# drscotthawley/flocoder

Hardware: NVIDIA B200
Metric: samples/sec, 50-step RK4 latent sampling (higher is better)
Workload: dtype bf16

## Files before the change

### flocoder_b200/csrc/api.cu

```cuda
#include <cuda_fp16.h>
#include <math.h>
#include <stdarg.h>
#include <stdio.h>
#include <stdlib.h>
#include <string.h>

#include <algorithm>
#include <chrono>
#include <float.h>
#include <map>
#include <memory>
#include <string>
#include <vector>

#include "flo_internal.h"

namespace flo {

int conv_umma_smem_bytes(const ConvUmmaParams& p);

static thread_local std::string g_last_error;
void set_error(const char* fmt, ...) {
    char buf[1024];
    va_list ap;
// ... 1535 lines not shown
        } else {
            snprintf(line, sizeof(line), "%3zu %-7s %-28s in=%s out_m=%s out_o=%s\n", i, kinds[op.kind], op.name.c_str(), bn(op.gn_in),
                     bn(op.out_m), bn(op.out_o));
            t += line;
        }
    }
    for (size_t i = 0; i < h.bufs.size(); ++i) {
        const Buf& bf = h.bufs[i];
        snprintf(line, sizeof(line), "buf %3zu %-34s C=%d %dx%d %s bytes_ps=%zu live=[%d,%d] off_ps=%zu\n", i, bf.name.c_str(), bf.C, bf.H,
                 bf.W, bf.bf16 ? "bf16" : "f32 ", bf.bytes_ps, bf.def, bf.last, bf.off_ps);
        t += line;
    }
    if (h.spec.fused) {
        FusedBuilder fb(h, h.ftensors, h.fstages, 4);
        rc = fb.build();
        if (rc) return rc;
        snprintf(line, sizeof(line), "fused: %d stages, %d boundary tensors, %zu bytes/sample\n", (int)h.fstages.size(),
                 (int)h.ftensors.size(), h.farena_ps);
        t += line;
        for (size_t i = 0; i < h.fstages.size(); ++i) {
            const FStage& st = h.fstages[i];
            if (st.kind == 0) {
                const ChainParams& c = st.cp;
                snprintf(line, sizeof(line), "stage %2zu chain %-12s %dx%d nb=%d mt=%d strips=%d steps=%d loads=%d smem=%d (slots %d, ring %dx%d) tmem=%d nsplit=%d ctas=%d\n",
                         i, st.name.c_str(), c.H, c.W, c.nb, c.n_mtiles, c.strips, c.n_steps, c.n_loads, c.smem_bytes, c.ring_off,
                         c.n_ring, c.ring_slot_bytes, c.tmem_cols, c.nsplit, c.nsplit * ((B + c.nb - 1) / c.nb));
                t += line;
                for (int k = 0; k < c.n_steps; ++k) {
                    const ChainStep& cs = c.st[k];
                    snprintf(line, sizeof(line), "      step %d: conv=%d k=%d cin=%d+%d n=%d chunks=%dx%d res=%d(%dx%d) epi=%d C=%d G=%d film=%d resmode=%d out_slot=%d out_g=%d un=%d up=%d pn=%d final=%d a0=%d a1=%d\n",
                             k, cs.has_conv, cs.ksize, cs.a0_ncb * 8, cs.a1_ncb * 8, cs.n, cs.slices, cs.slices_per_chunk, cs.has_res,
                             cs.res_slices, cs.res_slices_per_chunk, cs.epi, cs.C, cs.groups, cs.film_off, cs.res_mode, cs.out_slot_off,
                             cs.out_g, cs.out_un_g, cs.out_up_g, cs.pn_g, cs.final, cs.a0_off, cs.a1_off);
                    t += line;
                }
            } else {
                const AttnFusedParams& a = st.ap;
                snprintf(line, sizeof(line), "stage %2zu attn  %-12s %dx%d C=%d nb=%d n=%d n_pad=%d mt=%d full=%d smem=%d plane=%d tmem=%d cols(k=%d v=%d ctx=%d q=%d out=%d proj=%d) ctas=%d\n",
                         i, st.name.c_str(), a.H, a.W, a.C, a.nb, a.n, a.n_pad, a.n_mtiles, a.full, a.smem_bytes, a.plane_bytes, a.tmem_cols,
                         a.col_k, a.col_v, a.col_ctx, a.col_q, a.col_out, a.col_proj, (B + a.nb - 1) / a.nb);
                t += line;
            }
        }
        for (size_t i = 0; i < h.ftensors.size(); ++i) {
            snprintf(line, sizeof(line), "ftensor %2zu %-24s C=%d %dx%d off_ps=%zu\n", i, h.ftensors[i].name.c_str(), h.ftensors[i].C,
                     h.ftensors[i].H, h.ftensors[i].W, h.ftensors[i].off_ps);
            t += line;
        }
    }
    if (out && cap > 0) snprintf(out, cap, "%s", t.c_str());
    return (int)t.size();
}

static void op_cost(const Handle& h, const Op& op, double& fl, double& by) {
    const Spec& s = h.spec;
// ... 212 lines not shown
```

### flocoder_b200/csrc/flo_internal.h

```cpp
#pragma once
#include <cuda_runtime.h>
#include <cuda_bf16.h>
#include <cuda.h>
#include <stdint.h>
#include <string>
#include <vector>

#include "../../include/flocoder_b200.h"

namespace flo {

enum StageKind : int {
    ST_PLAIN = 0,
    ST_RK1 = 1,
    ST_RK2 = 2,
    ST_RK3 = 3,
    ST_RK4 = 4,
    ST_EULER = 5,
    ST_CFG_COND = 6,
    ST_STORE = 7
};
enum StageFlags : int {
    SF_CFG_COMBINE = 1,
    SF_CFG_2B = 2
// ... 169 lines not shown
size_t pack_umma_weights(const float* w_oihw, int cout, int cin, int ksize, const int* perm, int n_tile, bool f16,
                         std::vector<__nv_bfloat16>& out);

typedef CUresult (*EncodeTiledFn)(CUtensorMap*, CUtensorMapDataType, cuuint32_t, void*, const cuuint64_t*,
                                  const cuuint64_t*, const cuuint32_t*, const cuuint32_t*, CUtensorMapInterleave,
                                  CUtensorMapSwizzle, CUtensorMapL2promotion, CUtensorMapFloatOOBfill);
EncodeTiledFn get_encode_tiled();

void set_error(const char* fmt, ...);

constexpr int MAX_WSTAGES = 8;
constexpr int CH_MAX_STEPS = 8;
constexpr int CH_MAX_LOADS = 4;
constexpr int CH_MAX_GT = 10;
enum ChainEpi : int { CE_GN = 1, CE_BIAS = 2, CE_INIT = 3 };

struct ChainStep {
    int has_conv;
    int a0_off, a0_ncb, a1_off, a1_ncb;
    int ksize, n;
    int acc_col;
    unsigned w_off; int slices, slices_per_chunk;
    int has_res, res_col; unsigned wres_off; int res_slices, res_slices_per_chunk;
    int tab_idx, res_tab_idx;
    int chunk0, res_chunk0;
    int epi;
    int C, groups, silu, film_off;
    int bias_off, gamma_off, beta_off;
    int res_mode;
    int res_slot_off, res_bias_off;
    int out_slot_off;
    int out_g, out_un_g, out_up_g;
    int pn_g, pn_gamma_off, pn_beta_off;
    int final;
};

struct ChainParams {
    int n_steps;
    ChainStep st[CH_MAX_STEPS];
    int B, H, W, nb, n_mtiles, strips, plane_px;
    int n_loads, load_off[CH_MAX_LOADS], load_ncb[CH_MAX_LOADS];
    int zero_off, zero_bytes;
    int ones_off;
    int fast;
    int max_c;
    int g_max, coef_n, cpar_n;
    int wide;
    int ring_off, ring_slot_bytes, n_ring, n_ring_deep;
    int stats_off, bar_off, smem_bytes, tmem_cols;
    int tab_off, tab_n;
    int wtab_off, n_chunks;
    int tabs_off;
    int nsplit;
    int xpart_off;
    int fmt;
    int film_dim;
    int cin0, dim, channels;
    int init_w_off, init_b_off, final_w_off, final_b_off;
    const uint16_t* wblob;
    const float* fblob;
    void* gt[CH_MAX_GT];
    Ctrl* ctrl;
    long long* dbg;
};

struct AttnFusedParams {
    int epi_warps;
    int B, H, W, C, nb, n, n_pad, n_mtiles;
    int full;
    int ktrans;
    int small;
    int fmt;
    unsigned wq_off, wk_off, wv_off, wo_off;
    int qkv_chunks, qkv_S, o_chunks, o_S;
    int bo_off, gamma_off, beta_off;
    int xh_off, p_off, v_off, ct_off, kmax_off, stats_off;
    int plane_bytes;
// ... 54 lines not shown
```

### flocoder_b200/csrc/fused.cu

```cuda
#include <cuda_fp16.h>

#include <cstring>
#include <type_traits>
#include "flo_internal.h"
#include "umma_common.cuh"
#include "fused_common.cuh"

namespace flo {

struct Geo {
    int W, H, Wp, PP, nb, B, strips, sbo_px, tx_n;
};
__device__ __forceinline__ Geo make_geo(const ChainParams& p) {
    Geo g;
    g.W = p.W; g.H = p.H; g.Wp = p.W + 2; g.PP = g.Wp * (p.H + 2); g.nb = p.nb; g.B = p.B;
    g.strips = p.strips; g.sbo_px = p.strips ? g.Wp : 8; g.tx_n = p.W >> 3;
    return g;
}
__device__ __forceinline__ int tile_row0(const Geo& g, int t) {
    if (g.strips) return ((t / g.tx_n) * 16 + 1) * g.Wp + 1 + 8 * (t % g.tx_n);
    return g.Wp + 1 + t * 128;
}
struct RowInfo {
    int pp;
    int s, px;
    bool valid;
};
__device__ __forceinline__ RowInfo make_row(const Geo& g, int t, int r, int b0) {
    RowInfo ri;
    ri.pp = tile_row0(g, t) + (r >> 3) * g.sbo_px + (r & 7);
    ri.s = ri.pp / g.PP;
    const int rem = ri.pp - ri.s * g.PP;
    const int hh = rem / g.Wp, ww = rem - hh * g.Wp;
    ri.px = (hh - 1) * g.W + (ww - 1);
    ri.valid = (ri.s < g.nb) && (b0 + ri.s < g.B) && hh >= 1 && hh <= g.H && ww >= 1 && ww <= g.W;
    return ri;
}

struct RingPos {
    int slot; uint32_t phase;
    __device__ __forceinline__ void next(int n_ring) { if (++slot == n_ring) { slot = 0; phase ^= 1u; } }
};
struct ConvIssue {
    const int32_t* tab;
    int n, col, slices, S;
};
template <int MT>
struct IssueCtx {
    uint32_t tmem_base, bar_full, bar_empty, ring_lo, ring_slot16, ones_lo;
    uint32_t plane16;
    uint32_t desc_hi_a, desc_hi_ones;
    int n_ring;
    uint32_t row0[MT];
    int cc;
    RingPos rp;
    long long* dbg;
};
__device__ __forceinline__ uint64_t desc64(uint32_t lo, uint32_t hi) {
    uint64_t d;
    asm("mov.b64 %0, {%1, %2};" : "=l"(d) : "r"(lo), "r"(hi));
    return d;
}
template <int MT, int FMT>
__device__ __forceinline__ void issue_conv(IssueCtx<MT>& x, const ConvIssue& c) {
    const uint32_t idesc = make_idesc16(128, c.n, FMT, 0, 0);
    const uint32_t b_hi = (128u >> 4) | (1u << 14);
    const uint32_t b_lbo = ((uint32_t)c.n & 0x3FFFu) << 16;
    const uint32_t a_lbo = (x.plane16 & 0x3FFFu) << 16;
    const uint32_t slice16 = (uint32_t)c.n * 2u;
    const int conv_slices = c.slices - 1;
    for (int ks0 = 0; ks0 < c.slices; ks0 += c.S) {
        const int cnt = min(c.S, c.slices - ks0);
        const int slot = x.rp.slot;
        mbar_wait(x.bar_full + 8 * slot, x.rp.phase);
        tc_fence_after();
        if (x.dbg && x.cc >= 8 && x.cc < 16 && (threadIdx.x & 31) == 0) x.dbg[104 + (x.cc - 8) * 3 + 2] = clock64();
        if (elect_one()) {
            uint32_t b_lo = (x.ring_lo + (uint32_t)slot * x.ring_slot16) | b_lbo;
            const int32_t* tp = c.tab + ks0;
            const int n_conv = min(cnt, conv_slices - ks0);
            uint32_t acc = ks0 > 0 ? 1u : 0u;
            auto mma_slice = [&](int32_t e) {
                const uint64_t bdesc = desc64(b_lo, b_hi);
                const uint32_t a_base = (uint32_t)e | a_lbo;
#pragma unroll
                for (int t = 0; t < MT; ++t)
                    umma_bf16(x.tmem_base + (uint32_t)(c.col + t * c.n), desc64(a_base + x.row0[t], x.desc_hi_a), bdesc, idesc, acc);
                acc = 1u;
                b_lo += slice16;
            };
            int s = 0;
            if constexpr (MT == 1) {
                int32_t e[4], f[4];
#pragma unroll
                for (int k = 0; k < 4; ++k) e[k] = (n_conv >= 4) ? tp[k] : 0;
                for (; s + 4 <= n_conv; s += 4) {
#pragma unroll
                    for (int k = 0; k < 4; ++k) f[k] = (s + 8 <= n_conv) ? tp[s + 4 + k] : 0;
#pragma unroll
                    for (int k = 0; k < 4; ++k) mma_slice(e[k]);
#pragma unroll
                    for (int k = 0; k < 4; ++k) e[k] = f[k];
                }
            } else {
                int32_t cur = n_conv > 0 ? tp[0] : 0;
                for (; s < n_conv; ++s) {
                    const int32_t nxt = tp[s + 1];
                    mma_slice(cur);
                    cur = nxt;
                }
            }
            for (; s < n_conv; ++s) mma_slice(tp[s]);
            if (ks0 + cnt == c.slices) {
                const uint64_t bdesc = desc64(b_lo, b_hi);
                const uint64_t adesc = desc64(x.ones_lo | (8u << 16), x.desc_hi_ones);
#pragma unroll
                for (int t = 0; t < MT; ++t) umma_bf16(x.tmem_base + (uint32_t)(c.col + t * c.n), adesc, bdesc, idesc, 1u);
            }
            umma_commit(x.bar_empty + 8 * slot);
        }
        __syncwarp();
        ++x.cc;
        x.rp.next(x.n_ring);
    }
}

template <int N> struct IntTag { static constexpr int value = N; };

struct XChg {
    int nsplit; uint32_t rank, smem_base, bar_x; int xpart_off; uint32_t* phase; uint8_t* smem;
};
__device__ __forceinline__ void stats_to_coef(const Geo& g, int R, const float2* rowstat, float2* coef, const float2* gpar, int G, int pm,
                                              int C, int HW, bool has_film, int et, const XChg* xc = nullptr) {
    const int lgG = 31 - __clz(G), combos = g.nb * G, cpg = C >> lgG, GS = G * pm;
    const int cpw = (combos + EPI_WARPS - 1) / EPI_WARPS;
    int seg = 32;
// ... 57 lines not shown
        }
    }
    epi_sync();
}

template <int NV>
__device__ __forceinline__ int warp_sum_scatter(float (&p)[NV], int lane) {
    int idx = 0, o = 16;
#pragma unroll
    for (int h = NV / 2; h >= 1; h >>= 1, o >>= 1) {
        const bool upper = (lane & o) != 0;
#pragma unroll
        for (int j = 0; j < h; ++j) {
            const float send = upper ? p[j] : p[j + h];
            const float keep = upper ? p[j + h] : p[j];
            p[j] = keep + __shfl_xor_sync(0xffffffffu, send, o);
        }
        idx += upper ? h : 0;
    }
    for (; o >= 1; o >>= 1) p[0] += __shfl_xor_sync(0xffffffffu, p[0], o);
    return idx;
}

#ifndef FLO_CHAIN_MINB
#define FLO_CHAIN_MINB 2
#endif
constexpr int FINAL_MAX_CH = 4;
template <int MT, bool SPLIT, int FMT, bool FAST, bool WIDE = false, int ENDS = 3>
__global__ void __launch_bounds__(FUSED_THREADS, (MT <= 2 && !SPLIT && !WIDE) ? FLO_CHAIN_MINB : 1) k_chain(const __grid_constant__ CUtensorMap tm0,
                                                         const __grid_constant__ CUtensorMap tm1,
                                                         const __grid_constant__ CUtensorMap tm2,
                                                         const __grid_constant__ CUtensorMap tm3,
                                                         const __grid_constant__ ChainParams p) {
    extern __shared__ __align__(128) uint8_t smem[];
    const int warp = threadIdx.x >> 5, lane = threadIdx.x & 31, tid = threadIdx.x;
    constexpr int W_PROD = EPI_WARPS, W_MMA = EPI_WARPS + 1;
    const uint32_t smem_base = smem_u32(smem);
    const int bar_off = p.bar_off;
    const uint32_t bar_full = smem_base + bar_off;
    const uint32_t bar_empty = bar_full + 8 * MAX_WSTAGES;
    const uint32_t bar_load = bar_empty + 8 * MAX_WSTAGES;
    const uint32_t bar_mma = bar_load + 8;
    const uint32_t bar_epi = bar_mma + 8;
    const uint32_t tmem_slot = bar_epi + 8;
    const uint32_t bar_x = tmem_slot + 8;
    const uint32_t bar_epi2 = bar_x + 8;
    volatile uint32_t* tmem_slot_ptr = reinterpret_cast<volatile uint32_t*>(smem + bar_off + 16 * MAX_WSTAGES + 24);
    const Geo geo = make_geo(p);
    const int Q = SPLIT ? p.nsplit : 1;
    const uint32_t qrank = SPLIT ? cluster_ctarank() : 0u;
    const int lgQ = SPLIT ? 31 - __clz(Q) : 0;
    const int b0 = ((int)blockIdx.x >> lgQ) * geo.nb;
    const uint32_t plane_bytes = (uint32_t)p.plane_px * 16u;
    const int n_steps = p.n_steps, n_ring = p.n_ring, n_loads = p.n_loads, tmem_cols = p.tmem_cols;
    const int ones_off = p.ones_off;
    long long* dbg = (blockIdx.x == 0) ? p.dbg : nullptr;
    if (p.dbg && tid == 0 && blockIdx.x == 0) p.dbg[100] = global_ns();

    if (warp == W_PROD && lane == 0) {
        for (int i = 0; i < n_ring; ++i) { mbar_init(bar_full + 8 * i, 1); mbar_init(bar_empty + 8 * i, 1); }
        mbar_init(bar_load, 1);
        mbar_init(bar_mma, 1);
        mbar_init(bar_epi, SPLIT ? 1 : EPI_THREADS);
        mbar_init(bar_epi2, 1);
        mbar_init(bar_x, SPLIT ? 1 : EPI_THREADS);
        asm volatile("fence.mbarrier_init.release.cluster;" ::: "memory");
    }
    if (warp == W_MMA) tmem_alloc(tmem_slot, (uint32_t)tmem_cols);
    {
        const int zoff = p.zero_off, zbytes = p.zero_bytes;
        for (int i = tid * 16; i < zbytes; i += FUSED_THREADS * 16) *reinterpret_cast<uint4*>(smem + zoff + i) = make_uint4(0, 0, 0, 0);
        const uint32_t ones2 = pack2t<FMT>(1.0f, 1.0f);
        for (int i = tid; i < 256; i += FUSED_THREADS)
            *reinterpret_cast<uint4*>(smem + ones_off + i * 16) = make_uint4(i < 128 ? ones2 : 0u, 0, 0, 0);
    }
    int32_t* atab = reinterpret_cast<int32_t*>(smem + p.tab_off);
    {
        const int32_t* gtab = reinterpret_cast<const int32_t*>(p.fblob + p.tabs_off);
        const int base16 = (int)((smem_base >> 4) & 0x3FFFu);
        const int tab_n = p.tab_n, n_chunks = p.n_chunks;
        for (int i = tid; i < tab_n; i += FUSED_THREADS) atab[i] = gtab[i] + base16;
        const uint2* gw = reinterpret_cast<const uint2*>(gtab + tab_n) + (size_t)qrank * n_chunks;
        uint2* wtab_w = reinterpret_cast<uint2*>(smem + p.wtab_off);
        for (int i = tid; i < n_chunks; i += FUSED_THREADS) wtab_w[i] = gw[i];
    }
    fence_proxy_async();
    tc_fence_before();
    if (Q > 1) cluster_sync_all();
    else __syncthreads();
    tc_fence_after();
    const uint32_t tmem_base = *tmem_slot_ptr;
    if (dbg && tid == 0) dbg[CH_MAX_STEPS * 8] = clock64();
    if (dbg && tid == 0) dbg[101] = global_ns();

    if (warp == W_PROD) {
        if (dbg && lane == 8) {
            for (int cc = 0; cc < 16 && cc < p.n_chunks; ++cc) {
                mbar_wait(bar_full + 8 * (cc % n_ring), (uint32_t)(cc / n_ring) & 1u);
                if (cc >= 8) dbg[104 + (cc - 8) * 3] = clock64();
            }
        }
        constexpr int NL = 2;
        if (lane < NL) {
            const uint32_t ring_base = smem_base + p.ring_off, ring_slot_bytes = p.ring_slot_bytes;
            const uint2* wtab = reinterpret_cast<const uint2*>(smem + p.wtab_off);
// ... 29 lines not shown
        x.plane16 = plane_bytes >> 4;
        x.desc_hi_a = (((uint32_t)geo.sbo_px * 16u) >> 4) | (1u << 14);
        x.desc_hi_ones = (128u >> 4) | (1u << 14);
        x.n_ring = n_ring; x.cc = 0; x.rp.slot = 0; x.rp.phase = 0; x.dbg = dbg;
#pragma unroll
        for (int t = 0; t < MT; ++t) x.row0[t] = (uint32_t)(tile_row0(geo, t) - (geo.Wp + 1));
        if (n_loads > 0) mbar_wait(bar_load, 0);
        for (int i = 0; i < n_steps; ++i) {
            if (i > 0) {
                if (SPLIT) {
                    const int live = min(geo.nb, geo.B - b0) * geo.H * geo.W;
                    const uint32_t bar = ((i - 1) & 1) ? bar_epi2 : bar_epi;
                    if (elect_one()) mbar_expect_tx(bar, (uint32_t)(live * (p.st[i - 1].C >> 3) * 16));
                    __syncwarp();
                    mbar_wait_cluster(bar, ((i - 1) >> 1) & 1);
                    fence_proxy_async_all();
                } else {
                    named_bar_sync(2, EPI_THREADS + 32);
                }
            }
            tc_fence_after();
            if (dbg && lane == 0) dbg[i * 8 + 0] = clock64();
            if (p.st[i].has_conv) {
                ConvIssue c;
                c.tab = atab + p.st[i].tab_idx;
                c.n = p.st[i].n; c.col = p.st[i].acc_col; c.slices = p.st[i].slices;
                c.S = p.st[i].slices_per_chunk;
                issue_conv<MT, FMT>(x, c);
                if (p.st[i].has_res) {
                    c.tab = atab + p.st[i].res_tab_idx;
                    c.col = p.st[i].res_col; c.slices = p.st[i].res_slices; c.S = p.st[i].res_slices_per_chunk;
                    issue_conv<MT, FMT>(x, c);
                }
                if (dbg && lane == 0) dbg[i * 8 + 1] = clock64();
                if (elect_one()) umma_commit(bar_mma);
            } else {
                if (elect_one()) mbar_arrive(bar_mma);
            }
            __syncwarp();
        }
    } else {
        const int wg = warp >> 2, quad = warp & 3;
        const int r = quad * 32 + lane;
        const int et = tid;
        const uint32_t tlane = tmem_base + ((uint32_t)(quad * 32) << 16);
        float2* rowstat = reinterpret_cast<float2*>(smem + p.stats_off);
        float2* coef = rowstat + MT * 128 * p.g_max;
        float* cpar = reinterpret_cast<float*>(coef + p.coef_n);
        const int cpar_n = p.cpar_n;
        float2* gpar = reinterpret_cast<float2*>(cpar + cpar_n);
        float* const fastbuf = reinterpret_cast<float*>(gpar + p.max_c);
        Ctrl* ctrl = p.ctrl;
        const float* fblob = p.fblob;
        const int HW = geo.H * geo.W;
// ... 9 lines not shown
            const int t = (MT == 1) ? 0 : wg + 2 * k;
            if (t < MT) ri[k] = make_row(geo, t, r, b0);
            else { ri[k].pp = 0; ri[k].s = 0; ri[k].px = 0; ri[k].valid = false; }
        }
        if (n_loads > 0) mbar_wait(bar_load, 0);
        uint32_t xphase = 0;
        XChg xc;
        xc.nsplit = Q; xc.rank = qrank; xc.smem_base = smem_base; xc.bar_x = bar_x; xc.xpart_off = p.xpart_off; xc.phase = &xphase;
        xc.smem = smem;

        for (int i = 0; i < n_steps; ++i) {
            const int epi = p.st[i].epi, Ctot = p.st[i].C, acc_col = p.st[i].acc_col, res_col = p.st[i].res_col;
            const int C = Ctot >> lgQ, c0 = (int)qrank * C;
            const int res_mode = p.st[i].res_mode, res_slot_off = p.st[i].res_slot_off;
            const int is_final = (ENDS & 2) ? p.st[i].final : 0, pn_g = p.st[i].pn_g;
            const int out_slot_off = p.st[i].out_slot_off;
            uint4* const og = p.st[i].out_g >= 0 ? reinterpret_cast<uint4*>(p.gt[p.st[i].out_g]) : nullptr;
            int cbeg = 0, cend = C;
            if (MT == 1) {
                if (is_final) { cend = wg == 0 ? C : 0; }
                else { cbeg = wg * (C >> 1); cend = cbeg + (C >> 1); }
            }
            const bool cw8 = (cend - cbeg) == 8;
            auto write8 = [&](const RowInfo& R, int cb, const float* v8) -> uint4 {
                const uint4 u = pack8t<FMT>(v8);
                if (out_slot_off >= 0) {
                    const uint32_t soff = (uint32_t)out_slot_off + (uint32_t)cb * plane_bytes + (uint32_t)R.pp * 16u;
                    if (!SPLIT) *reinterpret_cast<uint4*>(smem + soff) = u;
                    else if (i + 1 < n_steps) {
                        const uint32_t bar = (i & 1) ? bar_epi2 : bar_epi;
                        for (int q = 0; q < Q; ++q) st_async_v4(mapa_shared(smem_base + soff, (uint32_t)q), u, mapa_shared(bar, (uint32_t)q));
                    } else {
                        *reinterpret_cast<uint4*>(smem + soff) = u;
                    }
                }
                if (og) og[(size_t)(cb * geo.B + b0 + R.s) * HW + R.px] = u;
                return u;
            };
            auto for_chunks = [&](auto&& fn) {
                if (cw8) {
                    fn(0, cbeg, IntTag<8>());
                } else {
#pragma unroll
                    for (int k = 0; k < TW; ++k) {
                        if (MT > 1 && wg + 2 * k >= MT) continue;
                        for (int c = cbeg; c < cend; c += 16) fn(k, c, IntTag<16>());
// ... 184 lines not shown
                    const int b = b0 + ri[k].s;
                    float xin[16];
#pragma unroll
                    for (int ci = 0; ci < 16; ++ci) xin[ci] = ci < cin0 ? xs[((size_t)b * cin0 + ci) * HW + ri[k].px] : 0.f;
                    for (int c8 = cbeg; c8 < cend; c8 += 8) {
                        float v[8];
#pragma unroll
                        for (int j = 0; j < 8; ++j) {
                            float a = cpar[C * cin0 + c8 + j];
                            if (cin0 == 4) {
                                const float4 w4 = *reinterpret_cast<const float4*>(cpar + (c8 + j) * 4);
                                a = fmaf(xin[0], w4.x, a); a = fmaf(xin[1], w4.y, a); a = fmaf(xin[2], w4.z, a); a = fmaf(xin[3], w4.w, a);
                            } else {
#pragma unroll
                                for (int ci = 0; ci < 16; ++ci)
                                    if (ci < cin0) a = fmaf(xin[ci], cpar[(c8 + j) * cin0 + ci], a);
                            }
                            v[j] = a;
                        }
                        write8(ri[k], (c0 + c8) >> 3, v);
                    }
                }
            } else if (epi == CE_BIAS) {
                for_chunks([&](int k, int c, auto tag) {
                    constexpr int CW = decltype(tag)::value;
                    uint32_t u[CW];
                    const uint32_t ta = tlane + (uint32_t)(acc_col + tile_of(k) * C + c);
                    if constexpr (CW == 16) tmem_ld16_issue(ta, u); else tmem_ld8_issue(ta, u);
                    tmem_ld_wait();
                    if (!ri[k].valid) return;
                    float v[CW];
#pragma unroll
                    for (int j = 0; j < CW; ++j) v[j] = __uint_as_float(u[j]);
#pragma unroll
                    for (int hb = 0; hb < CW / 8; ++hb) write8(ri[k], ((c0 + c) >> 3) + hb, v + hb * 8);
                });
            } else {
                const int G = p.st[i].groups >> lgQ, lg_cpg = 31 - __clz(C) - (31 - __clz(G)), cpg = 1 << lg_cpg;
                float kacc[TW][FINAL_MAX_CH];
                float psx[TW], psq[TW];
#pragma unroll
                for (int k = 0; k < TW; ++k) {
                    psx[k] = 0.f; psq[k] = 0.f;
#pragma unroll
                    for (int j = 0; j < FINAL_MAX_CH; ++j) kacc[k][j] = 0.f;
                }
                if constexpr (fast_gn_k) {
// ... 140 lines not shown
                                unpack8t<FMT>(pk[hb], xv);
                                const float4* pp4 = reinterpret_cast<const float4*>(pnpar + cbeg + hb * 8);
#pragma unroll
                                for (int j = 0; j < 8; j += 2) {
                                    const float4 gb = pp4[j >> 1];
                                    const float a0 = rstd * gb.x, a1 = rstd * gb.z;
                                    xv[j] = fmaf(xv[j], a0, gb.y - mean * a0); xv[j + 1] = fmaf(xv[j + 1], a1, gb.w - mean * a1);
                                }
                                dst[(size_t)(gcb * geo.B + b0) * HW + ri[0].px] = pack8t<FMT>(xv);
                            }
                        }
                    }
                } else {
                const int pm = (MT == 1 && G == 1 && !is_final) ? 2 : 1;
                const int GS = G * pm;
                bool fast2 = false;
                if constexpr (SPLIT && MT == 1)
                    fast2 = G == 1 && geo.PP == 16 && !is_final && (cend - cbeg == 8 || cend - cbeg == 16);
                bool fast3 = false;
                if constexpr (!SPLIT && MT == 1 && WIDE)
                    fast3 = geo.H == 4 && geo.W == 4 && geo.nb <= 3 && !is_final && (cpg == 8 || cpg == 16) && ((cend - cbeg) & 15) == 0 &&
                            cend > cbeg;
                if (fast2) {
                    if (dbg && et == 0) dbg[i * 8 + 3] = clock64();
                    auto body = [&](auto cw_tag) {
                        constexpr int CW = decltype(cw_tag)::value;
                        uint32_t av[CW];
                        const uint32_t ta = tlane + (uint32_t)(acc_col + cbeg);
                        if constexpr (CW == 16) tmem_ld16_issue(ta, av); else tmem_ld8_issue(ta, av);
                        tmem_ld_wait();
                        const bool valid = ri[0].valid;
                        float s0 = 0.f, q0 = 0.f, s1 = 0.f, q1 = 0.f;
#pragma unroll
                        for (int j = 0; j < CW; j += 2) {
                            const float xa = __uint_as_float(av[j]), xb = __uint_as_float(av[j + 1]);
                            s0 += xa; q0 = fmaf(xa, xa, q0); s1 += xb; q1 = fmaf(xb, xb, q1);
                        }
                        float sx = valid ? s0 + s1 : 0.f, sq = valid ? q0 + q1 : 0.f;
#pragma unroll
                        for (int o = 8; o > 0; o >>= 1) { sx += __shfl_xor_sync(0xffffffffu, sx, o); sq += __shfl_xor_sync(0xffffffffu, sq, o); }
                        float2* const part = reinterpret_cast<float2*>(fastbuf);
                        const int sl = r >> 4;
                        if ((lane & 15) == 0) part[wg * 8 + sl] = make_float2(sx, sq);
                        epi_sync();
                        if (dbg && et == 0) dbg[i * 8 + 4] = clock64();
                        uint32_t rv[CW];
                        if (res_mode == 1) {
                            const uint32_t tr = tlane + (uint32_t)(res_col + cbeg);
                            if constexpr (CW == 16) tmem_ld16_issue(tr, rv); else tmem_ld8_issue(tr, rv);
                            tmem_ld_wait();
                        }
                        if (!valid) return;
                        const float2 pa = part[sl], pb = part[8 + sl];
// ... 362 lines not shown
```

### flocoder_b200/csrc/fused_plan.inc

```

struct FusedBuilder {
    Handle& h;
    const Spec& s;
    std::vector<FTensor>& T;
    std::vector<FStage>& S;
    bool debug;
    int qcap;
    FusedBuilder(Handle& hh, std::vector<FTensor>& t, std::vector<FStage>& st, int qcap_)
        : h(hh), s(hh.spec), T(t), S(st), debug((hh.spec.flags & FLO_FLAG_NO_BUFFER_REUSE) != 0), qcap(qcap_) {}

    int tensor(const std::string& name, int C, int H, int W) {
        for (size_t i = 0; i < T.size(); ++i)
            if (T[i].name == name) return (int)i;
        FTensor t; t.name = name; t.C = C; t.H = H; t.W = W;
        t.bytes_ps = ((size_t)C * H * W * 2 + 255) & ~(size_t)255; t.off_ps = 0;
        T.push_back(t);
        return (int)T.size() - 1;
    }
    const Op& op(const std::string& name, int kind) {
        for (auto& o : h.ops)
            if (o.name == name && o.kind == kind) return o;
        set_error("internal: no op '%s'", name.c_str());
        throw 1;
    }
// ... 104 lines not shown
        }
        set_error("internal: global tensor table overflow in stage %s", cur.name.c_str());
        throw 1;
    }
    int load(int tensor_id) {
        const FTensor& t = T[tensor_id];
        const int off = slot(t.C);
        ChainParams& c = cur.cp;
        c.load_off[c.n_loads] = off; c.load_ncb[c.n_loads] = t.C / 8;
        cur.map_tensor[c.n_loads] = tensor_id;
        ++c.n_loads; cur.n_maps = c.n_loads;
        return off;
    }
    void mark_epi_slots() { if (first_epi_slot < 0) first_epi_slot = slot_top; }
    ChainStep& new_step() {
        ChainParams& c = cur.cp;
        if (c.n_steps >= CH_MAX_STEPS) { set_error("internal: too many steps in stage %s", cur.name.c_str()); throw 1; }
        ChainStep& st = c.st[c.n_steps++];
        memset(&st, 0, sizeof(st));
        st.film_off = -1; st.bias_off = -1; st.gamma_off = -1; st.beta_off = -1; st.res_slot_off = -1; st.res_bias_off = -1;
        st.out_slot_off = -1; st.out_g = -1; st.out_un_g = -1; st.out_up_g = -1; st.pn_g = -1;
        return st;
    }
    void set_conv(ChainStep& st, const Op& conv, int a0_off, int a0_C, int a1_off, int a1_C) {
        st.has_conv = 1;
        st.a0_off = a0_off; st.a0_ncb = a0_C / 8; st.a1_off = a1_off < 0 ? 0 : a1_off; st.a1_ncb = a1_off < 0 ? 0 : a1_C / 8;
        const int Q = cur.cp.nsplit, nq = conv.cout / Q;
        st.ksize = conv.ksize; st.n = nq; st.acc_col = 0;
        st.w_off = fused_stream(conv, Q);
        st.slices = conv.ksize * conv.ksize * (a0_C + (a1_off < 0 ? 0 : a1_C)) / 16 + 1;
        st.slices_per_chunk = chunk_slices(st.slices, nq);
        ring_slot = std::max(ring_slot, st.slices_per_chunk * nq * 32);
        max_n = std::max(max_n, nq);
        st.bias_off = -1;
        st.C = conv.cout;
    }
    int conv_bias(const std::string& opname, int a0_off, int a0_C, int C_out, int out_tensor = -1) {
        const Op& conv = op(opname, OP_CONV);
        mark_epi_slots();
        ChainStep& st = new_step();
        set_conv(st, conv, a0_off, a0_C, -1, 0);
        st.epi = CE_BIAS;
        st.out_slot_off = slot(C_out);
        st.out_g = gt(out_tensor);
        return st.out_slot_off;
    }
    int resblock(const std::string& p, int x0_off, int x0_C, int x1_off, int x1_C, int dout, int out_tensor, int pn_tensor,
                 bool is_final, int H, int W) {
        mark_epi_slots();
        const int cin = x0_C + (x1_off < 0 ? 0 : x1_C);
        const Op& c1 = op(p + ".block1.proj", OP_CONV);
        const Op& g1 = op(p + ".block1", OP_GN);
        if ((dout & (dout - 1)) || (g1.groups & (g1.groups - 1))) {
            set_error("fused path: channels (%d) and GroupNorm groups (%d) of '%s' must be powers of two", dout, g1.groups, p.c_str());
            throw 2;
        }
        const Op& c2 = op(p + ".block2.proj", OP_CONV);
        const Op& g2 = op(p, OP_GN);
        const bool has_res = cin != dout;
        const int hslot = slot(dout);
        {
            ChainStep& st = new_step();
            set_conv(st, c1, x0_off, x0_C, x1_off, x1_C);
            if (has_res) {
                const Op& rc = op(p + ".res_conv", OP_CONV);
                const int Q = cur.cp.nsplit;
                st.has_res = 1; st.wres_off = fused_stream(rc, Q);
                st.res_slices = cin / 16 + 1;
                st.res_slices_per_chunk = chunk_slices(st.res_slices, dout / Q);
                ring_slot = std::max(ring_slot, st.res_slices_per_chunk * (dout / Q) * 32);
            }
            st.epi = CE_GN; st.groups = g1.groups; st.silu = 1; st.film_off = g1.film_off;
            max_g = std::max(max_g, g1.groups); max_c = std::max(max_c, dout);
            st.gamma_off = (int)g1.gamma; st.beta_off = (int)g1.beta;
            st.out_slot_off = hslot;
            if (debug) st.out_g = gt(tensor(p + ".block1", dout, H, W));
        }
        int oslot = -1;
        {
            ChainStep& st = new_step();
            set_conv(st, c2, hslot, dout, -1, 0);
            st.epi = CE_GN; st.groups = g2.groups; st.silu = 1; st.film_off = -1;
            st.gamma_off = (int)g2.gamma; st.beta_off = (int)g2.beta;
            if (has_res) {
                st.res_mode = 1; st.res_bias_off = -1;
            } else {
                st.res_mode = 2; st.res_slot_off = x0_off;
            }
            if (is_final) {
                st.final = 1;
            } else {
                oslot = slot(dout);
                st.out_slot_off = oslot;
                st.out_g = gt(out_tensor);
                if (pn_tensor >= 0) {
                    const Op& pn = op(pn_name, OP_GN);
                    st.pn_g = gt(pn_tensor); st.pn_gamma_off = (int)pn.gamma; st.pn_beta_off = (int)pn.beta;
                }
            }
        }
        release(hslot, dout);
        return oslot;
    }
    std::string pn_name;
    int end_chain() {
        ChainParams& c = cur.cp;
        const int acc_cols = c.n_mtiles * max_n;
        bool any_res = false;
        for (int i = 0; i < c.n_steps; ++i) any_res |= c.st[i].has_res != 0;
        for (int i = 0; i < c.n_steps; ++i) {
            c.st[i].res_col = acc_cols;
            if (c.st[i].res_mode == 1) c.st[i].res_col = acc_cols;
        }
        int cols = 32;
        while (cols < acc_cols * (any_res ? 2 : 1)) cols <<= 1;
        if (cols > 512) { set_error("stage %s needs %d TMEM columns", cur.name.c_str(), cols); return FLO_ERR_UNSUPPORTED; }
        c.tmem_cols = cols;
        if (first_epi_slot < 0) first_epi_slot = slot_top;
        c.zero_off = first_epi_slot; c.zero_bytes = slot_top - first_epi_slot;
        const int Wp = c.W + 2;
        int off = (slot_top + (128 + Wp + 2) * 16 + 127) & ~127;
        c.ones_off = off; off += 4096;
        c.ring_slot_bytes = (ring_slot + 127) & ~127;
        c.g_max = std::max(max_g, 2); c.coef_n = c.nb * max_c;
        c.cpar_n = std::max(512, s.dim * (s.channels + 1));
        c.max_c = max_c;
        {
            bool fast = c.nb == 1 && c.n_mtiles <= 2 && c.nsplit == 1;
            for (int i = 0; i < c.n_steps && fast; ++i) {
                const int width = c.n_mtiles == 1 ? (c.st[i].final ? c.st[i].C : c.st[i].C / 2) : c.st[i].C;
                if (width > 16) fast = false;
            }
            c.fast = fast ? 1 : 0;
        }
        const int stats_bytes = (c.n_mtiles * 128 * c.g_max + c.coef_n) * 8 + c.cpar_n * 4 + max_c * 8 + 512 + 4 * max_c * 8;
        int tab_n = 0;
        for (int i = 0; i < c.n_steps; ++i) {
            if (!c.st[i].has_conv) continue;
            c.st[i].tab_idx = tab_n; tab_n += c.st[i].slices + 1;
            if (c.st[i].has_res) { c.st[i].res_tab_idx = tab_n; tab_n += c.st[i].res_slices + 1; }
        }
        c.tab_n = (tab_n + 3) & ~3;
        int n_chunks = 0;
        for (int i = 0; i < c.n_steps; ++i) {
            if (!c.st[i].has_conv) continue;
            c.st[i].chunk0 = n_chunks; n_chunks += (c.st[i].slices + c.st[i].slices_per_chunk - 1) / c.st[i].slices_per_chunk;
            if (c.st[i].has_res) {
                c.st[i].res_chunk0 = n_chunks;
                n_chunks += (c.st[i].res_slices + c.st[i].res_slices_per_chunk - 1) / c.st[i].res_slices_per_chunk;
            }
        }
        c.n_chunks = n_chunks;
        {
            std::vector<int32_t> tabs((size_t)c.tab_n + (size_t)c.nsplit * n_chunks * 2, 0);
            const int two_planes = (c.plane_px * 16 >> 4) * 2, Wp_ = c.W + 2;
            auto fill_a = [&](int idx, int conv_slices, int ksize, const ChainStep& st) {
                const int a0p = st.a0_ncb >> 1, pairs = a0p + (st.a1_ncb >> 1);
                for (int ks = 0; ks < conv_slices; ++ks) {
                    const int tap = ks / pairs, cp = ks - tap * pairs;
                    const int shift = (ksize == 3 ? ((tap / 3 - 1) * Wp_ + (tap % 3 - 1)) : 0) + Wp_ + 1;
                    const int plane = cp < a0p ? (st.a0_off >> 4) + cp * two_planes : (st.a1_off >> 4) + (cp - a0p) * two_planes;
                    tabs[(size_t)idx + ks] = plane + shift;
                }
            };
            auto fill_w = [&](int chunk0, unsigned w_off, int slices, int S, int n) {
                const int nch = (slices + S - 1) / S;
                for (int q = 0; q < c.nsplit; ++q)
                    for (int k = 0; k < nch; ++k) {
                        int32_t* e = &tabs[(size_t)c.tab_n + ((size_t)q * n_chunks + chunk0 + k) * 2];
                        e[0] = (int32_t)((w_off + (unsigned)q * (unsigned)(slices * n * 16)) * 2u + (unsigned)(k * S) * (unsigned)n * 32u);
                        e[1] = (int32_t)(std::min(S, slices - k * S) * n * 32);
                    }
            };
            for (int i = 0; i < c.n_steps; ++i) {
                const ChainStep& st = c.st[i];
                if (!st.has_conv) continue;
                fill_a(st.tab_idx, st.slices - 1, st.ksize, st);
                fill_w(st.chunk0, st.w_off, st.slices, st.slices_per_chunk, st.n);
                if (st.has_res) {
                    fill_a(st.res_tab_idx, st.res_slices - 1, 1, st);
                    fill_w(st.res_chunk0, st.wres_off, st.res_slices, st.res_slices_per_chunk, st.n);
                }
            }
            size_t boff = (h.blob_f32.size() + 7) & ~(size_t)7;
            h.blob_f32.resize(boff + tabs.size());
            memcpy(h.blob_f32.data() + boff, tabs.data(), tabs.size() * sizeof(int32_t));
            c.tabs_off = (int)boff;
        }
        const int xpart_bytes = (c.nsplit * c.nb * 8 + 15) & ~15;
        c.stats_off = off; off += stats_bytes;
        c.tab_off = off; off += c.tab_n * 4;
        c.wtab_off = off; off += ((c.n_chunks + 1) & ~1) * 8;
        c.xpart_off = off; off += xpart_bytes;
        c.bar_off = off; off += 16 * MAX_WSTAGES + 48;
        off = (off + 127) & ~127;
        c.ring_off = off;
        const int fixed = off;
        const int half_sm = 113 * 1024;
        const int cap = std::min(MAX_WSTAGES, std::max(2, c.n_chunks));
        c.n_ring_deep = std::min(cap, (227 * 1024 - fixed) / c.ring_slot_bytes);
        if (fixed + 2 * c.ring_slot_bytes <= half_sm) c.n_ring = std::min(std::min(4, cap), (half_sm - fixed) / c.ring_slot_bytes);
        else c.n_ring = c.n_ring_deep;
        if (c.n_ring < 2) { set_error("stage %s does not fit in shared memory (%d bytes before the weight ring)", cur.name.c_str(), fixed); return FLO_ERR_UNSUPPORTED; }
        off += c.n_ring * c.ring_slot_bytes;
        c.smem_bytes = off;
        S.push_back(cur);
        return FLO_OK;
    }

    int attention(const std::string& p, bool full, int C, int H, int W, int xhat_t, int x2_t, int out_t, int out_un_t,
                  int out_up_t) {
        FStage st;
        st.kind = 1; st.name = p; st.n_maps = 1; st.map_tensor[0] = xhat_t;
        for (int i = 0; i < CH_MAX_GT; ++i) st.gt_tensor[i] = -1;
        st.x2_t = x2_t; st.out_t = out_t; st.out_un_t = out_un_t; st.out_up_t = out_up_t;
        memset(&st.ap, 0, sizeof(st.ap));
        AttnFusedParams& a = st.ap;
// ... 301 lines not shown
```

Measured before the change: 4201.

## Add K-split convolution across cluster CTAs with DSMEM partial-sum exchange

For small 2x2 chain stages with a cluster split, convolutions can now be split along the reduction (K) dimension instead of output channels when a simple cost model favours it. Each CTA computes partial sums over its slice of K for all output channels, then the partials are exchanged through distributed shared memory with st.async and a cluster mbarrier and reduced in the epilogue, with only the last rank adding bias. This aims to cut per-CTA MMA instruction count for narrow-N layers, at the cost of extra shared memory for exchange slots, cross-CTA synchronisation, and per-rank A-operand tables.

```diff
diff --git a/flocoder_b200/csrc/api.cu b/flocoder_b200/csrc/api.cu
--- a/flocoder_b200/csrc/api.cu
+++ b/flocoder_b200/csrc/api.cu
@@ -1581,15 +1581,15 @@
             const FStage& st = h.fstages[i];
             if (st.kind == 0) {
                 const ChainParams& c = st.cp;
-                snprintf(line, sizeof(line), "stage %2zu chain %-12s %dx%d nb=%d mt=%d strips=%d steps=%d loads=%d smem=%d (slots %d, ring %dx%d) tmem=%d nsplit=%d ctas=%d\n",
+                snprintf(line, sizeof(line), "stage %2zu chain %-12s %dx%d nb=%d mt=%d strips=%d steps=%d loads=%d smem=%d (slots %d, ring %dx%d, kx %d) tmem=%d nsplit=%d ctas=%d\n",
                          i, st.name.c_str(), c.H, c.W, c.nb, c.n_mtiles, c.strips, c.n_steps, c.n_loads, c.smem_bytes, c.ring_off,
-                         c.n_ring, c.ring_slot_bytes, c.tmem_cols, c.nsplit, c.nsplit * ((B + c.nb - 1) / c.nb));
+                         c.n_ring, c.ring_slot_bytes, c.bar_off - c.kx_off, c.tmem_cols, c.nsplit, c.nsplit * ((B + c.nb - 1) / c.nb));
                 t += line;
                 for (int k = 0; k < c.n_steps; ++k) {
                     const ChainStep& cs = c.st[k];
-                    snprintf(line, sizeof(line), "      step %d: conv=%d k=%d cin=%d+%d n=%d chunks=%dx%d res=%d(%dx%d) epi=%d C=%d G=%d film=%d resmode=%d out_slot=%d out_g=%d un=%d up=%d pn=%d final=%d a0=%d a1=%d\n",
-                             k, cs.has_conv, cs.ksize, cs.a0_ncb * 8, cs.a1_ncb * 8, cs.n, cs.slices, cs.slices_per_chunk, cs.has_res,
-                             cs.res_slices, cs.res_slices_per_chunk, cs.epi, cs.C, cs.groups, cs.film_off, cs.res_mode, cs.out_slot_off,
+                    snprintf(line, sizeof(line), "      step %d: conv=%d k=%d cin=%d+%d ksplit=%d n=%d chunks=%dx%d res=%d(%dx%d n=%d) epi=%d C=%d G=%d film=%d resmode=%d out_slot=%d out_g=%d un=%d up=%d pn=%d final=%d a0=%d a1=%d\n",
+                             k, cs.has_conv, cs.ksize, cs.a0_ncb * 8, cs.a1_ncb * 8, cs.ksplit, cs.n, cs.slices, cs.slices_per_chunk, cs.has_res,
+                             cs.res_slices, cs.res_slices_per_chunk, cs.res_n, cs.epi, cs.C, cs.groups, cs.film_off, cs.res_mode, cs.out_slot_off,
                              cs.out_g, cs.out_un_g, cs.out_up_g, cs.pn_g, cs.final, cs.a0_off, cs.a1_off);
                     t += line;
                 }
diff --git a/flocoder_b200/csrc/flo_internal.h b/flocoder_b200/csrc/flo_internal.h
--- a/flocoder_b200/csrc/flo_internal.h
+++ b/flocoder_b200/csrc/flo_internal.h
@@ -215,6 +215,9 @@
     int acc_col;
     unsigned w_off; int slices, slices_per_chunk;
     int has_res, res_col; unsigned wres_off; int res_slices, res_slices_per_chunk;
+    int res_n;
+    int ksplit;
+    int kx_parity;
     int tab_idx, res_tab_idx;
     int chunk0, res_chunk0;
     int epi;
@@ -246,6 +249,7 @@
     int tabs_off;
     int nsplit;
     int xpart_off;
+    int kx_off;
     int fmt;
     int film_dim;
     int cin0, dim, channels;
diff --git a/flocoder_b200/csrc/fused.cu b/flocoder_b200/csrc/fused.cu
--- a/flocoder_b200/csrc/fused.cu
+++ b/flocoder_b200/csrc/fused.cu
@@ -44,6 +44,7 @@
 struct ConvIssue {
     const int32_t* tab;
     int n, col, slices, S;
+    int bias;
 };
 template <int MT>
 struct IssueCtx {
@@ -68,7 +69,7 @@
     const uint32_t b_lbo = ((uint32_t)c.n & 0x3FFFu) << 16;
     const uint32_t a_lbo = (x.plane16 & 0x3FFFu) << 16;
     const uint32_t slice16 = (uint32_t)c.n * 2u;
-    const int conv_slices = c.slices - 1;
+    const int conv_slices = c.slices - c.bias;
     for (int ks0 = 0; ks0 < c.slices; ks0 += c.S) {
         const int cnt = min(c.S, c.slices - ks0);
         const int slot = x.rp.slot;
@@ -111,7 +112,7 @@
                 }
             }
             for (; s < n_conv; ++s) mma_slice(tp[s]);
-            if (ks0 + cnt == c.slices) {
+            if (c.bias && ks0 + cnt == c.slices) {
                 const uint64_t bdesc = desc64(b_lo, b_hi);
                 const uint64_t adesc = desc64(x.ones_lo | (8u << 16), x.desc_hi_ones);
 #pragma unroll
@@ -215,6 +216,56 @@
     return idx;
 }
 
+struct KxArgs {
+    uint32_t tcol;
+    int C, Q, rank;
+    bool valid;
+    uint32_t row_off;
+    uint32_t slot_bytes;
+    uint32_t kx_off, smem_base; const uint8_t* smem;
+    uint32_t bar;
+    uint32_t expect;
+    uint32_t parity;
+};
+template <int CW>
+__device__ __forceinline__ void kx_reduce(uint32_t (&av)[CW], const KxArgs& a) {
+    if (a.expect) mbar_expect_tx(a.bar, a.expect);
+    auto slot_off = [&](int owner, int sender) { return a.kx_off + (uint32_t)(sender - (sender > owner ? 1 : 0)) * a.slot_bytes + a.row_off; };
+    for (int k = 1; k < a.Q; ++k) {
+        const int q = (a.rank + k) & (a.Q - 1);
+        uint32_t u[CW];
+        if constexpr (CW == 16) tmem_ld16_issue(a.tcol + (uint32_t)(q * a.C), u); else tmem_ld8_issue(a.tcol + (uint32_t)(q * a.C), u);
+        tmem_ld_wait();
+        if (a.valid) {
+            const uint32_t dst = mapa_shared(a.smem_base + slot_off(q, a.rank), (uint32_t)q), rbar = mapa_shared(a.bar, (uint32_t)q);
+#pragma unroll
+            for (int j = 0; j < CW; j += 4) st_async_v4(dst + (uint32_t)j * 4u, make_uint4(u[j], u[j + 1], u[j + 2], u[j + 3]), rbar);
+        }
+    }
+    if constexpr (CW == 16) tmem_ld16_issue(a.tcol + (uint32_t)(a.rank * a.C), av); else tmem_ld8_issue(a.tcol + (uint32_t)(a.rank * a.C), av);
+    tmem_ld_wait();
+    mbar_wait_cluster(a.bar, a.parity);
+    if (!a.valid) return;
+    float sum[CW];
+#pragma unroll
+    for (int q = 0; q < 4; ++q) {
+        if (q >= a.Q) continue;
+        float v[CW];
+        if (q == a.rank) {
+#pragma unroll
+            for (int j = 0; j < CW; ++j) v[j] = __uint_as_float(av[j]);
+        } else {
+            const float4* src = reinterpret_cast<const float4*>(a.smem + slot_off(a.rank, q));
+#pragma unroll
+            for (int j = 0; j < CW; j += 4) { const float4 f = src[j >> 2]; v[j] = f.x; v[j + 1] = f.y; v[j + 2] = f.z; v[j + 3] = f.w; }
+        }
+#pragma unroll
+        for (int j = 0; j < CW; ++j) sum[j] = q == 0 ? v[j] : sum[j] + v[j];
+    }
+#pragma unroll
+    for (int j = 0; j < CW; ++j) av[j] = __float_as_uint(sum[j]);
+}
+
 #ifndef FLO_CHAIN_MINB
 #define FLO_CHAIN_MINB 2
 #endif
@@ -238,6 +289,7 @@
     const uint32_t tmem_slot = bar_epi + 8;
     const uint32_t bar_x = tmem_slot + 8;
     const uint32_t bar_epi2 = bar_x + 8;
+    const uint32_t bar_kx = bar_epi2 + 8;
     volatile uint32_t* tmem_slot_ptr = reinterpret_cast<volatile uint32_t*>(smem + bar_off + 16 * MAX_WSTAGES + 24);
     const Geo geo = make_geo(p);
     const int Q = SPLIT ? p.nsplit : 1;
@@ -256,6 +308,7 @@
         mbar_init(bar_mma, 1);
         mbar_init(bar_epi, SPLIT ? 1 : EPI_THREADS);
         mbar_init(bar_epi2, 1);
+        mbar_init(bar_kx, 1);
         mbar_init(bar_x, SPLIT ? 1 : EPI_THREADS);
         asm volatile("fence.mbarrier_init.release.cluster;" ::: "memory");
     }
@@ -272,8 +325,9 @@
         const int32_t* gtab = reinterpret_cast<const int32_t*>(p.fblob + p.tabs_off);
         const int base16 = (int)((smem_base >> 4) & 0x3FFFu);
         const int tab_n = p.tab_n, n_chunks = p.n_chunks;
-        for (int i = tid; i < tab_n; i += FUSED_THREADS) atab[i] = gtab[i] + base16;
-        const uint2* gw = reinterpret_cast<const uint2*>(gtab + tab_n) + (size_t)qrank * n_chunks;
+        const int32_t* ga = gtab + (size_t)qrank * tab_n;
+        for (int i = tid; i < tab_n; i += FUSED_THREADS) atab[i] = ga[i] + base16;
+        const uint2* gw = reinterpret_cast<const uint2*>(gtab + (size_t)Q * tab_n) + (size_t)qrank * n_chunks;
         uint2* wtab_w = reinterpret_cast<uint2*>(smem + p.wtab_off);
         for (int i = tid; i < n_chunks; i += FUSED_THREADS) wtab_w[i] = gw[i];
     }
@@ -349,14 +403,16 @@
             tc_fence_after();
             if (dbg && lane == 0) dbg[i * 8 + 0] = clock64();
             if (p.st[i].has_conv) {
+                const int no_bias = (SPLIT && p.st[i].ksplit && (int)qrank != Q - 1) ? 1 : 0;
                 ConvIssue c;
                 c.tab = atab + p.st[i].tab_idx;
-                c.n = p.st[i].n; c.col = p.st[i].acc_col; c.slices = p.st[i].slices;
+                c.n = p.st[i].n; c.col = p.st[i].acc_col; c.slices = p.st[i].slices - no_bias; c.bias = 1 - no_bias;
                 c.S = p.st[i].slices_per_chunk;
                 issue_conv<MT, FMT>(x, c);
                 if (p.st[i].has_res) {
                     c.tab = atab + p.st[i].res_tab_idx;
-                    c.col = p.st[i].res_col; c.slices = p.st[i].res_slices; c.S = p.st[i].res_slices_per_chunk;
+                    c.n = p.st[i].res_n; c.col = p.st[i].res_col; c.slices = p.st[i].res_slices; c.bias = 1;
+                    c.S = p.st[i].res_slices_per_chunk;
                     issue_conv<MT, FMT>(x, c);
                 }
                 if (dbg && lane == 0) dbg[i * 8 + 1] = clock64();
@@ -412,6 +468,16 @@
                 else { cbeg = wg * (C >> 1); cend = cbeg + (C >> 1); }
             }
             const bool cw8 = (cend - cbeg) == 8;
+            const bool ksplit = SPLIT && p.st[i].ksplit;
+            auto kx_args = [&]() {
+                KxArgs a;
+                a.tcol = tlane + (uint32_t)(acc_col + cbeg); a.C = C; a.Q = Q; a.rank = (int)qrank; a.valid = ri[0].valid;
+                a.row_off = (uint32_t)(((ri[0].s * HW + ri[0].px) * C + cbeg) * 4); a.slot_bytes = (uint32_t)(geo.nb * HW * C * 4);
+                a.kx_off = (uint32_t)p.kx_off; a.smem_base = smem_base; a.smem = smem; a.bar = bar_kx;
+                a.expect = et == 0 ? (uint32_t)((Q - 1) * min(geo.nb, geo.B - b0) * HW * C * 4) : 0u;
+                a.parity = (uint32_t)p.st[i].kx_parity;
+                return a;
+            };
             auto write8 = [&](const RowInfo& R, int cb, const float* v8) -> uint4 {
                 const uint4 u = pack8t<FMT>(v8);
                 if (out_slot_off >= 0) {
@@ -642,7 +708,24 @@
                     }
                 }
             } else if (epi == CE_BIAS) {
-                for_chunks([&](int k, int c, auto tag) {
+                if constexpr (SPLIT && MT == 1) {
+                    if (ksplit) {
+                        auto kbias = [&](auto cw_tag) {
+                            constexpr int CW = decltype(cw_tag)::value;
+                            uint32_t av[CW];
+                            kx_reduce(av, kx_args());
+                            if (dbg && et == 0) { dbg[i * 8 + 3] = clock64(); dbg[i * 8 + 4] = dbg[i * 8 + 3]; }
+                            if (!ri[0].valid) return;
+                            float v[CW];
+#pragma unroll
+                            for (int j = 0; j < CW; ++j) v[j] = __uint_as_float(av[j]);
+#pragma unroll
+                            for (int hb = 0; hb < CW / 8; ++hb) write8(ri[0], ((c0 + cbeg) >> 3) + hb, v + hb * 8);
+                        };
+                        if (cw8) kbias(IntTag<8>()); else kbias(IntTag<16>());
+                    }
+                }
+                if (!ksplit) for_chunks([&](int k, int c, auto tag) {
                     constexpr int CW = decltype(tag)::value;
                     uint32_t u[CW];
                     const uint32_t ta = tlane + (uint32_t)(acc_col + tile_of(k) * C + c);
@@ -829,13 +912,21 @@
                     fast3 = geo.H == 4 && geo.W == 4 && geo.nb <= 3 && !is_final && (cpg == 8 || cpg == 16) && ((cend - cbeg) & 15) == 0 &&
                             cend > cbeg;
                 if (fast2) {
-                    if (dbg && et == 0) dbg[i * 8 + 3] = clock64();
+                    if (dbg && et == 0 && !ksplit) dbg[i * 8 + 3] = clock64();
                     auto body = [&](auto cw_tag) {
                         constexpr int CW = decltype(cw_tag)::value;
                         uint32_t av[CW];
-                        const uint32_t ta = tlane + (uint32_t)(acc_col + cbeg);
-                        if constexpr (CW == 16) tmem_ld16_issue(ta, av); else tmem_ld8_issue(ta, av);
-                        tmem_ld_wait();
+                        if constexpr (SPLIT && MT == 1) {
+                            if (ksplit) {
+                                kx_reduce(av, kx_args());
+                                if (dbg && et == 0) dbg[i * 8 + 3] = clock64();
+                            }
+                        }
+                        if (!ksplit) {
+                            const uint32_t ta = tlane + (uint32_t)(acc_col + cbeg);
+                            if constexpr (CW == 16) tmem_ld16_issue(ta, av); else tmem_ld8_issue(ta, av);
+                            tmem_ld_wait();
+                        }
                         const bool valid = ri[0].valid;
                         float s0 = 0.f, q0 = 0.f, s1 = 0.f, q1 = 0.f;
 #pragma unroll
diff --git a/flocoder_b200/csrc/fused_plan.inc b/flocoder_b200/csrc/fused_plan.inc
--- a/flocoder_b200/csrc/fused_plan.inc
+++ b/flocoder_b200/csrc/fused_plan.inc
@@ -150,16 +150,32 @@
         st.out_slot_off = -1; st.out_g = -1; st.out_un_g = -1; st.out_up_g = -1; st.pn_g = -1;
         return st;
     }
-    void set_conv(ChainStep& st, const Op& conv, int a0_off, int a0_C, int a1_off, int a1_C) {
+    int ksplit_chunk(int kq, int n) const {
+        int S = chunk_slices(kq + 1, n);
+        while (S > 1 && kq % S == 0) --S;
+        return S > 1 ? S : 0;
+    }
+    bool ksplit_wins(const Op& conv, int cin, int gn_groups) const {
+        const ChainParams& c = cur.cp;
+        const int Q = c.nsplit, C = conv.cout, K = conv.ksize * conv.ksize * cin / 16;
+        if (Q == 1 || c.H != 2 || c.W != 2 || c.n_mtiles != 1) return false;
+        if ((C / Q != 16 && C / Q != 32) || (gn_groups > 0 && gn_groups != Q)) return false;
+        if (K % Q || !ksplit_chunk(K / Q, C)) return false;
+        auto mma = [](int instr, int n) { return instr * (4096.0 + n * 32.0) / 80.0; };
+        const double kx_cycles = 1000.0;
+        return mma(K / Q + 1, C) + kx_cycles < mma(K + 1, C / Q);
+    }
+    void set_conv(ChainStep& st, const Op& conv, int a0_off, int a0_C, int a1_off, int a1_C, bool ks = false) {
         st.has_conv = 1;
         st.a0_off = a0_off; st.a0_ncb = a0_C / 8; st.a1_off = a1_off < 0 ? 0 : a1_off; st.a1_ncb = a1_off < 0 ? 0 : a1_C / 8;
-        const int Q = cur.cp.nsplit, nq = conv.cout / Q;
-        st.ksize = conv.ksize; st.n = nq; st.acc_col = 0;
-        st.w_off = fused_stream(conv, Q);
-        st.slices = conv.ksize * conv.ksize * (a0_C + (a1_off < 0 ? 0 : a1_C)) / 16 + 1;
-        st.slices_per_chunk = chunk_slices(st.slices, nq);
-        ring_slot = std::max(ring_slot, st.slices_per_chunk * nq * 32);
-        max_n = std::max(max_n, nq);
+        const int Q = cur.cp.nsplit, n = ks ? conv.cout : conv.cout / Q;
+        const int K = conv.ksize * conv.ksize * (a0_C + (a1_off < 0 ? 0 : a1_C)) / 16;
+        st.ksize = conv.ksize; st.n = n; st.acc_col = 0; st.ksplit = ks ? 1 : 0;
+        st.w_off = fused_stream(conv, ks ? 1 : Q);
+        st.slices = (ks ? K / Q : K) + 1;
+        st.slices_per_chunk = ks ? ksplit_chunk(K / Q, n) : chunk_slices(st.slices, n);
+        ring_slot = std::max(ring_slot, st.slices_per_chunk * n * 32);
+        max_n = std::max(max_n, n);
         st.bias_off = -1;
         st.C = conv.cout;
     }
@@ -167,7 +183,7 @@
         const Op& conv = op(opname, OP_CONV);
         mark_epi_slots();
         ChainStep& st = new_step();
-        set_conv(st, conv, a0_off, a0_C, -1, 0);
+        set_conv(st, conv, a0_off, a0_C, -1, 0, ksplit_wins(conv, a0_C, 0));
         st.epi = CE_BIAS;
         st.out_slot_off = slot(C_out);
         st.out_g = gt(out_tensor);
@@ -189,14 +205,14 @@
         const int hslot = slot(dout);
         {
             ChainStep& st = new_step();
-            set_conv(st, c1, x0_off, x0_C, x1_off, x1_C);
+            set_conv(st, c1, x0_off, x0_C, x1_off, x1_C, ksplit_wins(c1, cin, g1.groups));
             if (has_res) {
                 const Op& rc = op(p + ".res_conv", OP_CONV);
                 const int Q = cur.cp.nsplit;
-                st.has_res = 1; st.wres_off = fused_stream(rc, Q);
+                st.has_res = 1; st.wres_off = fused_stream(rc, Q); st.res_n = dout / Q;
                 st.res_slices = cin / 16 + 1;
-                st.res_slices_per_chunk = chunk_slices(st.res_slices, dout / Q);
-                ring_slot = std::max(ring_slot, st.res_slices_per_chunk * (dout / Q) * 32);
+                st.res_slices_per_chunk = chunk_slices(st.res_slices, st.res_n);
+                ring_slot = std::max(ring_slot, st.res_slices_per_chunk * st.res_n * 32);
             }
             st.epi = CE_GN; st.groups = g1.groups; st.silu = 1; st.film_off = g1.film_off;
             max_g = std::max(max_g, g1.groups); max_c = std::max(max_c, dout);
@@ -207,7 +223,7 @@
         int oslot = -1;
         {
             ChainStep& st = new_step();
-            set_conv(st, c2, hslot, dout, -1, 0);
+            set_conv(st, c2, hslot, dout, -1, 0, !is_final && ksplit_wins(c2, dout, g2.groups));
             st.epi = CE_GN; st.groups = g2.groups; st.silu = 1; st.film_off = -1;
             st.gamma_off = (int)g2.gamma; st.beta_off = (int)g2.beta;
             if (has_res) {
@@ -250,9 +266,10 @@
         int off = (slot_top + (128 + Wp + 2) * 16 + 127) & ~127;
         c.ones_off = off; off += 4096;
         c.ring_slot_bytes = (ring_slot + 127) & ~127;
-        c.g_max = std::max(max_g, 2); c.coef_n = c.nb * max_c;
+        const int cta_c = std::max(max_c / c.nsplit, 16);
+        c.g_max = std::max(max_g, 2); c.coef_n = c.nb * cta_c;
         c.cpar_n = std::max(512, s.dim * (s.channels + 1));
-        c.max_c = max_c;
+        c.max_c = cta_c;
         {
             bool fast = c.nb == 1 && c.n_mtiles <= 2 && c.nsplit == 1;
             for (int i = 0; i < c.n_steps && fast; ++i) {
@@ -261,7 +278,7 @@
             }
             c.fast = fast ? 1 : 0;
         }
-        const int stats_bytes = (c.n_mtiles * 128 * c.g_max + c.coef_n) * 8 + c.cpar_n * 4 + max_c * 8 + 512 + 4 * max_c * 8;
+        const int stats_bytes = (c.n_mtiles * 128 * c.g_max + c.coef_n) * 8 + c.cpar_n * 4 + cta_c * 8 + 512 + 4 * cta_c * 8;
         int tab_n = 0;
         for (int i = 0; i < c.n_steps; ++i) {
             if (!c.st[i].has_conv) continue;
@@ -280,35 +297,41 @@
         }
         c.n_chunks = n_chunks;
         {
-            std::vector<int32_t> tabs((size_t)c.tab_n + (size_t)c.nsplit * n_chunks * 2, 0);
+            const int Q = c.nsplit;
+            std::vector<int32_t> tabs((size_t)Q * c.tab_n + (size_t)Q * n_chunks * 2, 0);
             const int two_planes = (c.plane_px * 16 >> 4) * 2, Wp_ = c.W + 2;
-            auto fill_a = [&](int idx, int conv_slices, int ksize, const ChainStep& st) {
+            auto fill_a = [&](int q, int idx, int ks0, int cnt, int ksize, const ChainStep& st) {
                 const int a0p = st.a0_ncb >> 1, pairs = a0p + (st.a1_ncb >> 1);
-                for (int ks = 0; ks < conv_slices; ++ks) {
-                    const int tap = ks / pairs, cp = ks - tap * pairs;
+                for (int k = 0; k < cnt; ++k) {
+                    const int ks = ks0 + k, tap = ks / pairs, cp = ks - tap * pairs;
                     const int shift = (ksize == 3 ? ((tap / 3 - 1) * Wp_ + (tap % 3 - 1)) : 0) + Wp_ + 1;
                     const int plane = cp < a0p ? (st.a0_off >> 4) + cp * two_planes : (st.a1_off >> 4) + (cp - a0p) * two_planes;
-                    tabs[(size_t)idx + ks] = plane + shift;
+                    tabs[(size_t)q * c.tab_n + idx + k] = plane + shift;
                 }
             };
-            auto fill_w = [&](int chunk0, unsigned w_off, int slices, int S, int n) {
+            auto fill_w = [&](int chunk0, unsigned w_off, int slices, int S, int n, bool ks) {
                 const int nch = (slices + S - 1) / S;
-                for (int q = 0; q < c.nsplit; ++q)
+                for (int q = 0; q < Q; ++q) {
+                    const int cnt = ks && q != Q - 1 ? slices - 1 : slices;
+                    const unsigned base = ks ? w_off * 2u + (unsigned)(q * (slices - 1)) * (unsigned)n * 32u
+                                             : (w_off + (unsigned)q * (unsigned)(slices * n * 16)) * 2u;
                     for (int k = 0; k < nch; ++k) {
-                        int32_t* e = &tabs[(size_t)c.tab_n + ((size_t)q * n_chunks + chunk0 + k) * 2];
-                        e[0] = (int32_t)((w_off + (unsigned)q * (unsigned)(slices * n * 16)) * 2u + (unsigned)(k * S) * (unsigned)n * 32u);
-                        e[1] = (int32_t)(std::min(S, slices - k * S) * n * 32);
+                        int32_t* e = &tabs[(size_t)Q * c.tab_n + ((size_t)q * n_chunks + chunk0 + k) * 2];
+                        e[0] = (int32_t)(base + (unsigned)(k * S) * (unsigned)n * 32u);
+                        e[1] = (int32_t)(std::min(S, cnt - k * S) * n * 32);
                     }
+                }
             };
             for (int i = 0; i < c.n_steps; ++i) {
                 const ChainStep& st = c.st[i];
                 if (!st.has_conv) continue;
-                fill_a(st.tab_idx, st.slices - 1, st.ksize, st);
-                fill_w(st.chunk0, st.w_off, st.slices, st.slices_per_chunk, st.n);
-                if (st.has_res) {
-                    fill_a(st.res_tab_idx, st.res_slices - 1, 1, st);
-                    fill_w(st.res_chunk0, st.wres_off, st.res_slices, st.res_slices_per_chunk, st.n);
+                const int kq = st.ksplit ? st.slices - 1 : 0;
+                for (int q = 0; q < Q; ++q) {
+                    fill_a(q, st.tab_idx, q * kq, st.ksplit ? kq : st.slices - 1, st.ksize, st);
+                    if (st.has_res) fill_a(q, st.res_tab_idx, 0, st.res_slices - 1, 1, st);
                 }
+                fill_w(st.chunk0, st.w_off, st.slices, st.slices_per_chunk, st.n, st.ksplit != 0);
+                if (st.has_res) fill_w(st.res_chunk0, st.wres_off, st.res_slices, st.res_slices_per_chunk, st.res_n, false);
             }
             size_t boff = (h.blob_f32.size() + 7) & ~(size_t)7;
             h.blob_f32.resize(boff + tabs.size());
@@ -316,11 +339,18 @@
             c.tabs_off = (int)boff;
         }
         const int xpart_bytes = (c.nsplit * c.nb * 8 + 15) & ~15;
+        int kx_bytes = 0, kx_steps = 0;
+        for (int i = 0; i < c.n_steps; ++i)
+            if (c.st[i].ksplit) {
+                kx_bytes = std::max(kx_bytes, (c.nsplit - 1) * c.nb * c.H * c.W * (c.st[i].C / c.nsplit) * 4);
+                c.st[i].kx_parity = kx_steps++ & 1;
+            }
         c.stats_off = off; off += stats_bytes;
         c.tab_off = off; off += c.tab_n * 4;
         c.wtab_off = off; off += ((c.n_chunks + 1) & ~1) * 8;
         c.xpart_off = off; off += xpart_bytes;
-        c.bar_off = off; off += 16 * MAX_WSTAGES + 48;
+        c.kx_off = off; off += kx_bytes;
+        c.bar_off = off; off += 16 * MAX_WSTAGES + 64;
         off = (off + 127) & ~127;
         c.ring_off = off;
         const int fixed = off;
```

Result: slower. 4071 (median of 6 runs) (-3.1%).
